# mjq11302010044/TPGSR

Hardware: AMD Instinct MI355X
Metric: training img/s (16x64->32x128, bs=48/GPU), TPGSR-TSRN full train step (higher is better)
Workload: dtype bf16x2; 1 GPU; C3: TPGSR-TSRN = TSRN_TL (STN+mask) + CRNN teacher/student text prior, stu_iter 1, full train step (teacher fwd, student fwd+bwd, distill loss, prior dropout, SR fwd+bwd, ImageLoss(gradient), clip 0.25, Adam); tpg=crnn, batch_per_gpu=48, global_batch=48, parallelism=dp1, launch=recorded plans, plain launches: main + weight-gradient + teacher streams

## Files before the change

### tpgsr_amd/csrc/conv_halo3.hip

```cpp
#include "conv_xbf_common.h"
#include <type_traits>

__device__ unsigned long long* g_halo3_trace = nullptr;
#define H3_STAMP(slot)                                                                                       \
  do {                                                                                                       \
    if (trace && lane == 0 && (slot) < 256)                                                                  \
      __builtin_nontemporal_store((unsigned long long)wall_clock64(), trace + (blockIdx.x * 8 + wave) * 256 + (slot)); \
  } while (0)

#define H3_TM 3
#define H3_NE 15
#define H3_PLANE (32 * H3_NE * 64)

template <int LD, int T, int TAPS>
__global__ __launch_bounds__(512, 2) void conv_halo3_xbf_kernel(tpgsr_conv_args a, int M, int Lcap) {
  extern __shared__ __attribute__((aligned(16))) unsigned char hsm[];
  constexpr int PLANE = H3_PLANE, BUF = T * PLANE;
  float* red_base = reinterpret_cast<float*>(hsm + 2 * BUF);
  float* stage_base = red_base + 2 * H3_TM * 256;
  const int tid = threadIdx.x;
  const int lane = tid & 63, wave = __builtin_amdgcn_readfirstlane(tid >> 6);
  typedef __attribute__((address_space(1))) unsigned long long* gptr_t;
  const gptr_t trace = blockIdx.x < 8 ? (gptr_t)g_halo3_trace : (gptr_t) nullptr;
  H3_STAMP(255);
  const int nbn = (a.Cout + 63) >> 6;
  const int mtiles = (M + 63) >> 6;
  const int nst = ((mtiles + H3_TM - 1) / H3_TM) * nbn;
  const int taps = a.KH * a.KW, NC = a.Cin >> 5;
  const int Hp = a.OH + a.KH - 1, Wp = a.OW + a.KW - 1, ohw = a.OH * a.OW;
  auto qbase = [&](int m) __attribute__((always_inline)) {
    const int n = m / ohw, r = m - n * ohw, oh = r / a.OW;
    return (n * Hp + oh) * Wp + (r - oh * a.OW);
  };

  if (wave >= 4) {
    const int pt = tid - 256, aq = pt & 7, er = pt >> 3;
    const __amdgpu_buffer_rsrc_t rs_in = make_rsrc(a.in, (size_t)a.N * a.H * a.W * a.in_ld);
    const __amdgpu_buffer_rsrc_t rs_in2 = make_rsrc(a.in2 ? a.in2 : a.in, (size_t)a.N * a.H * a.W * a.in2_ld);
    int hpix[H3_NE];
    auto decode_tile = [&](const int t) __attribute__((always_inline)) {
      const int m0 = (xcd_remap(t, nst) / nbn) * (64 * H3_TM);
      const int q0 = qbase(m0);
      const int L = qbase(min(m0 + 64 * H3_TM - 1, M - 1)) - q0 + (a.KH - 1) * Wp + a.KW;
      const int q = q0 + er * H3_NE;
      int n = q / (Hp * Wp);
      const int rem = q - n * (Hp * Wp);
      int r = rem / Wp, sx = rem - r * Wp;
#pragma unroll
      for (int i = 0; i < H3_NE; ++i) {
        const int ih = r - a.pad_h, iw = sx - a.pad_w;
        const bool in = n < a.N && (unsigned)ih < (unsigned)a.H && (unsigned)iw < (unsigned)a.W;
        hpix[i] = er * H3_NE + i < L ? (in ? (n * a.H + ih) * a.W + iw : -1) : -2;
        const bool c1 = ++sx >= Wp;
        sx = c1 ? 0 : sx;
        r += c1 ? 1 : 0;
        const bool c2 = r >= Hp;
        r = c2 ? 0 : r;
        n += c2 ? 1 : 0;
      }
    };
    constexpr bool DB = !(LD & 4);
    ARaw hr[DB ? 2 : 1][H3_NE];
    float4 qs[2], qt[2], q2 = make_float4(1.f, 1.f, 1.f, 1.f);
    qs[0] = qs[1] = make_float4(1.f, 1.f, 1.f, 1.f);
    qt[0] = qt[1] = make_float4(0.f, 0.f, 0.f, 0.f);
    auto load_item = [&](auto set_tag, const int cc) __attribute__((always_inline)) {
      constexpr int S = decltype(set_tag)::value;
      const int c = cc * 32 + aq * 4;
#pragma unroll
      for (int i = 0; i < H3_NE; ++i) {
        const bool ok = hpix[i] >= 0;
        hr[S][i].ok = (LD & 3) ? ok : true;
        hr[S][i].raw = false;
        hr[S][i].v = buf_load4(rs_in, ok ? ((unsigned)hpix[i] * (unsigned)a.in_ld + (unsigned)(a.in_coff + c)) * 4u : OOB_OFF);
        if (LD & 4) hr[S][i].v2 = buf_load4(rs_in2, ok ? ((unsigned)hpix[i] * (unsigned)a.in2_ld + (unsigned)c) * 4u : OOB_OFF);
      }
      if (LD & 1) {
        qs[S] = *reinterpret_cast<const float4*>(a.in_scale + c);
        qt[S] = *reinterpret_cast<const float4*>(a.in_shift + c);
      }
      if (LD & 32) q2 = *reinterpret_cast<const float4*>(a.in2_scale + c);
    };
    auto store_item = [&](auto set_tag, const int j) __attribute__((always_inline)) {
      constexpr int S = decltype(set_tag)::value;
      unsigned char* buf = hsm + (j & 1) * BUF;
#pragma unroll
      for (int i = 0; i < H3_NE; ++i) {
        const float4 v = finish_a<LD>(a, hr[S][i], qs[S], qt[S], q2);
        uint2 h[T];
        split4<T>(v, h);
        const int e = er * H3_NE + i;
        const int off = e * 64 + (((aq >> 1) ^ ((e >> 2) & 3)) << 4) + (aq & 1) * 8;
#pragma unroll
        for (int t = 0; t < T; ++t) *reinterpret_cast<uint2*>(buf + t * PLANE + off) = h[t];
      }
    };
    int t = blockIdx.x, cc = 0, j = 0;
    using P0 = std::integral_constant<int, 0>;
    using PN = std::integral_constant<int, DB ? 1 : 0>;
    decode_tile(t);
    if (DB) load_item(P0{}, 0);
    auto item = [&](auto cur_tag, auto nxt_tag) __attribute__((always_inline)) -> bool {
      int ncc = cc + 1, nt = t;
      if (ncc == NC) {
        ncc = 0;
        nt = t + gridDim.x;
      }
      const bool more = nt < nst;
      if (!DB) load_item(cur_tag, cc);
      if (more && ncc == 0) decode_tile(nt);
      if (DB && more) load_item(nxt_tag, ncc);
      H3_STAMP(4 * j);
      store_item(cur_tag, j);
      H3_STAMP(4 * j + 1);
      __syncthreads();
      H3_STAMP(4 * j + 2);
      ++j;
      t = nt;
      cc = ncc;
      return more;
    };
    while (true) {
      if (!item(P0{}, PN{})) break;
      if (!item(PN{}, P0{})) break;
    }
    __syncthreads();
    return;
  }

  {
  const int wm = wave & 1, wn = wave >> 1;
  const int wrows = a.wt_ld > 0 ? a.wt_ld : a.Cout;
  const int NB32 = (wrows + 31) >> 5, KB16 = a.kp >> 4;
  const __amdgpu_buffer_rsrc_t rs_w = make_rsrc(reinterpret_cast<const float*>(a.wt_bf), (size_t)T * NB32 * 32 * a.kp / 2);
  const unsigned plane_w = (unsigned)NB32 * KB16 * 1024u;
  const int g = lane >> 5;
  unsigned woff = 0;
  int ebase[H3_TM];

  floatx16 acc[H3_TM][1][1];
  bf16x8 av[2][H3_TM][T];
  u32x4 bw[2][2][T];
  int gtap = 0;
  auto fetch_w = [&](auto set_tag, auto kb_tag, const int tapidx) __attribute__((always_inline)) {
    constexpr int S = decltype(set_tag)::value, KB = decltype(kb_tag)::value;
#pragma unroll
    for (int t = 0; t < T; ++t)
      bw[S][KB][t] = __builtin_amdgcn_raw_buffer_load_b128(rs_w, (int)woff, (int)(t * plane_w + (unsigned)(2 * tapidx + KB) * 1024u), 0);
  };
  int an[H3_TM];
  auto addr_a = [&](auto kb_tag, const int bufoff, const int tapoff) __attribute__((always_inline)) {
    constexpr int KB = decltype(kb_tag)::value;
#pragma unroll
    for (int m = 0; m < H3_TM; ++m) {
      const int e = ebase[m] + tapoff;
      an[m] = bufoff + e * 64 + (((KB * 2 + g) ^ ((e >> 2) & 3)) << 4);
    }
  };
  auto read_a = [&](auto kb_tag) __attribute__((always_inline)) {
    constexpr int KB = decltype(kb_tag)::value;
#pragma unroll
    for (int m = 0; m < H3_TM; ++m)
#pragma unroll
      for (int t = 0; t < T; ++t) av[KB][m][t] = *reinterpret_cast<const bf16x8*>(hsm + an[m] + t * PLANE);
  };
  auto multiply = [&](auto set_tag, auto kb_tag) __attribute__((always_inline)) {
    constexpr int S = decltype(set_tag)::value, KB = decltype(kb_tag)::value;
    bf16x8 bv[T];
#pragma unroll
    for (int t = 0; t < T; ++t) bv[t] = __builtin_bit_cast(bf16x8, bw[S][KB][t]);
    if (T == 2) {
#pragma unroll
      for (int m = 0; m < H3_TM; ++m) acc[m][0][0] = __builtin_amdgcn_mfma_f32_32x32x16_bf16(av[KB][m][0], bv[T - 1], acc[m][0][0], 0, 0, 0);
#pragma unroll
      for (int m = 0; m < H3_TM; ++m) acc[m][0][0] = __builtin_amdgcn_mfma_f32_32x32x16_bf16(av[KB][m][T - 1], bv[0], acc[m][0][0], 0, 0, 0);
    }
#pragma unroll
    for (int m = 0; m < H3_TM; ++m) acc[m][0][0] = __builtin_amdgcn_mfma_f32_32x32x16_bf16(av[KB][m][0], bv[0], acc[m][0][0], 0, 0, 0);
  };
  using I0 = std::integral_constant<int, 0>;
  using I1 = std::integral_constant<int, 1>;
  int kw = 0, tapoff = 0;
  auto next_tap = [&]() __attribute__((always_inline)) {
    const bool cw = ++kw == a.KW;
    tapoff += cw ? Wp - a.KW + 1 : 1;
    kw = cw ? 0 : kw;
    asm volatile("" : "+s"(tapoff));
  };
#define H3_SGB(mask, n) __builtin_amdgcn_sched_group_barrier(mask, n, 0)
  auto interleave = [&](const bool ds) __attribute__((always_inline)) {
    constexpr int NM = 3 * (2 * T - 1);
    int used = 0;
    if (ds) {
#pragma unroll
      for (int i = 0; i < 3; ++i) {
        H3_SGB(0x008, 1);
        H3_SGB(0x100, T);
      }
      used = 3;
    }
    H3_SGB(0x008, 1);
    H3_SGB(0x020, T);
    ++used;
#pragma unroll
    for (int i = 0; i < NM; ++i) {
      if (i >= NM - used) break;
      H3_SGB(0x008, 1);
      H3_SGB(0x002, 3);
    }
  };
  auto tap = [&](auto set_tag, auto next_tag, const int bufoff) __attribute__((always_inline)) {
    constexpr int S = decltype(set_tag)::value;
    constexpr bool NEXT = decltype(next_tag)::value != 0;
    using SX = std::integral_constant<int, S ^ 1>;
    __builtin_amdgcn_sched_barrier(0);
    read_a(I1{});
    fetch_w(SX{}, I1{}, gtap + 1);
    if (NEXT) {
      next_tap();
      addr_a(I0{}, bufoff, tapoff);
    }
    multiply(set_tag, I0{});
    interleave(true);
    __builtin_amdgcn_sched_barrier(0);
    if (NEXT) read_a(I0{});
    fetch_w(set_tag, I0{}, gtap + 2);
    if (NEXT) addr_a(I1{}, bufoff, tapoff);
    multiply(set_tag, I1{});
    interleave(NEXT);
    __builtin_amdgcn_sched_barrier(0);
    ++gtap;
  };
  auto run_block = [&](auto s0_tag, const int bufoff) __attribute__((always_inline)) {
    constexpr int S0 = decltype(s0_tag)::value;
    using A0 = std::integral_constant<int, S0>;
    using A1 = std::integral_constant<int, S0 ^ 1>;
    kw = 0;
    tapoff = 0;
    addr_a(I0{}, bufoff, 0);
    read_a(I0{});
    addr_a(I1{}, bufoff, 0);
    if constexpr (TAPS > 0) {
      auto unrolled = [&](auto seq) __attribute__((always_inline)) {
        [&]<int... I>(std::integer_sequence<int, I...>) __attribute__((always_inline)) {
          (tap(std::integral_constant<int, S0 ^ (I & 1)>{}, std::integral_constant<int, (I + 1 < TAPS) ? 1 : 0>{}, bufoff), ...);
        }(seq);
      };
      unrolled(std::make_integer_sequence<int, TAPS>{});
    } else {
      for (int tp = 0; tp + 2 < taps; tp += 2) {
        tap(A0{}, I1{}, bufoff);
        tap(A1{}, I1{}, bufoff);
      }
      tap(A0{}, I0{}, bufoff);
    }
  };
  int j = 0, pend_mblk = -1, pend_n0 = 0, ndone = 0;
  auto flush_pending = [&]() __attribute__((always_inline)) {
    if (pend_mblk >= 0) {
      if (a.bn_row_tiles == H3_TM) {
        if (tid < 64 && pend_n0 + tid < a.Cout) {
          float v0 = 0.f, v1 = 0.f;
#pragma unroll
          for (int m = 0; m < H3_TM; ++m)
            if ((pend_mblk + m) * 64 < M) {
              const float* red = red_base + (((ndone - 1) & 1) * H3_TM + m) * 256;
              v0 += red[tid] + red[128 + tid];
              v1 += red[64 + tid] + red[192 + tid];
            }
          float* dst = a.bn_partial + (size_t)(pend_mblk / H3_TM) * 2 * a.Cout;
          dst[pend_n0 + tid] = v0;
          dst[a.Cout + pend_n0 + tid] = v1;
        }
      } else {
#pragma unroll
        for (int m = 0; m < H3_TM; ++m)
          if ((pend_mblk + m) * 64 < M)
            xbf_bn_flush<1, 1>(a, M, pend_n0, pend_mblk + m, tid, red_base + (((ndone - 1) & 1) * H3_TM + m) * 256);
      }
      pend_mblk = -1;
    }
  };
  for (int st = blockIdx.x; st < nst; st += gridDim.x) {
    const int tile = xcd_remap(st, nst);
    const int mblk3 = tile / nbn;
    const int m0 = mblk3 * (64 * H3_TM), n0 = (tile - mblk3 * nbn) * 64;
    const int q0 = qbase(m0);
    const int ncol0 = n0 + wn * 32;
    woff = ncol0 < a.Cout ? ((unsigned)((a.wt_coff + ncol0) >> 5) * KB16) * 1024u + lane * 16u : OOB_OFF;
#pragma unroll
    for (int m = 0; m < H3_TM; ++m) {
      ebase[m] = qbase(min(m0 + 64 * m + wm * 32 + (lane & 31), M - 1)) - q0;
#pragma unroll
      for (int r = 0; r < 16; ++r) acc[m][0][0][r] = 0.f;
    }
    gtap = 0;
    fetch_w(I0{}, I0{}, 0);
    fetch_w(I0{}, I1{}, 0);
    fetch_w(I1{}, I0{}, 1);
    for (int cc = 0; cc < NC; cc += 2) {
      H3_STAMP(4 * j);
      __syncthreads();
      H3_STAMP(4 * j + 1);
      flush_pending();
      run_block(I0{}, (j & 1) * BUF);
      H3_STAMP(4 * j + 2);
      ++j;
      if (cc + 1 < NC) {
        H3_STAMP(4 * j);
        __syncthreads();
        H3_STAMP(4 * j + 1);
        run_block(I1{}, (j & 1) * BUF);
        H3_STAMP(4 * j + 2);
        ++j;
      }
    }
    const bool bnb = a.bnb_y != nullptr;
    const bool fast = !a.out_ps && (a.Cout & 3) == 0 && (a.out_ld & 3) == 0 && (a.out_coff & 3) == 0 && ((uintptr_t)a.out & 15) == 0 &&
                      (!bnb || ((uintptr_t)a.bnb_y & 15) == 0);
    const bool full3 = m0 + 64 * (H3_TM - 1) < M;
    if (fast && !bnb && a.out_act == TPGSR_ACT_NONE && full3) {
      const int cloc = wn * 32 + (lane & 31), n = n0 + cloc;
      const bool nvalid = n < a.Cout;
      const float bias = (a.bias && nvalid) ? a.bias[n] : 0.f;
      const int quad = lane & 7, nq = n0 + wn * 32 + quad * 4;
      auto stage = [&](auto m_tag, float* stg) __attribute__((always_inline)) {
        constexpr int m = decltype(m_tag)::value;
        float sum = 0.f, sq = 0.f;
#pragma unroll
        for (int r = 0; r < 16; ++r) {
          const float raw = acc[m][0][0][r];
          if (nvalid) {
            sum += raw;
            sq = __builtin_fmaf(raw, raw, sq);
          }
          stg[((r & 3) + 8 * (r >> 2) + 4 * (lane >> 5)) * 32 + (lane & 31)] = raw + bias;
        }
        if (a.bn_partial) {
          float* red = red_base + ((ndone & 1) * H3_TM + m) * 256;
          sum += __shfl_xor(sum, 32);
          sq += __shfl_xor(sq, 32);
          if (lane < 32) {
            red[(wm * 2 + 0) * 64 + cloc] = sum;
            red[(wm * 2 + 1) * 64 + cloc] = sq;
          }
        }
      };
      auto drain = [&](auto m_tag, const float* stg) __attribute__((always_inline)) {
        constexpr int m = decltype(m_tag)::value;
#pragma unroll
        for (int k = 0; k < 4; ++k) {
          const int row = 8 * k + (lane >> 3);
          const float4 q4 = *reinterpret_cast<const float4*>(stg + row * 32 + quad * 4);
          if (nq < a.Cout) *reinterpret_cast<float4*>(a.out + (size_t)(m0 + 64 * m + wm * 32 + row) * a.out_ld + a.out_coff + nq) = q4;
        }
      };
      float* s0 = stage_base + wave * 2048;
      float* s1 = s0 + 1024;
      using M0 = std::integral_constant<int, 0>;
      using M1 = std::integral_constant<int, 1>;
      using M2 = std::integral_constant<int, 2>;
      stage(M0{}, s0);
      stage(M1{}, s1);
      drain(M0{}, s0);
      stage(M2{}, s0);
      drain(M1{}, s1);
      drain(M2{}, s0);
    } else {
    const int cloc = wn * 32 + (lane & 31), n = n0 + cloc;
    const bool nvalid = n < a.Cout;
    const float bias = (a.bias && nvalid) ? a.bias[n] : 0.f;
    const int quad = lane & 7, nq = n0 + wn * 32 + quad * 4;
    float b_mu = 0.f, b_rs = 0.f, b_sc = 1.f, b_sh = 0.f;
    if (bnb && nvalid) {
      if (a.bn_partial) {
        b_mu = a.bnb_mean[n];
        b_rs = a.bnb_rstd[n];
      }
      if (a.bnb_act && a.bnb_scale) {
        b_sc = a.bnb_scale[n];
        b_sh = a.bnb_shift[n];
      }
    }
    float4 yq[4];
    auto load_y = [&](const int m, float4 (&dst)[4]) __attribute__((always_inline)) {
#pragma unroll
      for (int k = 0; k < 4; ++k) {
        const int mm = m0 + 64 * m + wm * 32 + 8 * k + (lane >> 3);
        dst[k] = (mm < M && nq < a.Cout) ? *reinterpret_cast<const float4*>(a.bnb_y + (size_t)mm * a.Cout + nq) : make_float4(0.f, 0.f, 0.f, 0.f);
      }
    };
    if (bnb && fast) load_y(0, yq);
#pragma clang loop unroll(disable)
    for (int m = 0; m < H3_TM; ++m) {
      if (m0 + 64 * m >= M) break;
      floatx16 tile[1][1];
#pragma unroll
      for (int r = 0; r < 16; ++r) tile[0][0][r] = m == 0 ? acc[0][0][0][r] : m == 1 ? acc[1][0][0][r] : acc[2][0][0][r];
      float* red = red_base + ((ndone & 1) * H3_TM + m) * 256;
      if (!fast) {
        xbf_store_tile<1, 1>(a, tile, M, m0 + 64 * m, n0, wm, wn, lane, red);
        continue;
      }
      float* stg = stage_base + wave * 2048;
      float yv[16];
      float4 ynx[4];
      if (bnb) {
        if (m + 1 < H3_TM) load_y(m + 1, ynx);
#pragma unroll
        for (int k = 0; k < 4; ++k) *reinterpret_cast<float4*>(stg + (8 * k + (lane >> 3)) * 32 + quad * 4) = yq[k];
#pragma unroll
        for (int r = 0; r < 16; ++r) yv[r] = stg[((r & 3) + 8 * (r >> 2) + 4 * (lane >> 5)) * 32 + (lane & 31)];
      }
      float sum = 0.f, sq = 0.f;
      float v[16];
#pragma unroll
      for (int r = 0; r < 16; ++r) {
        const int row = (r & 3) + 8 * (r >> 2) + 4 * (lane >> 5);
        const int mm = m0 + 64 * m + wm * 32 + row;
        float raw = tile[0][0][r];
        if (mm < M && nvalid) {
          if (bnb) {
            const float dz = xbf_bnb_elem(raw, yv[r], b_sc, b_sh, b_mu, b_rs, a.bnb_act, sum, sq);
            if (a.bnb_store_dz) raw = dz;
          } else {
            sum += raw;
            sq = __builtin_fmaf(raw, raw, sq);
          }
        }
        v[r] = raw + bias;
      }
      if (a.out_act != TPGSR_ACT_NONE) {
#pragma unroll
        for (int r = 0; r < 16; ++r) v[r] = apply_act(v[r], a.out_act);
      }
#pragma unroll
      for (int r = 0; r < 16; ++r) stg[((r & 3) + 8 * (r >> 2) + 4 * (lane >> 5)) * 32 + (lane & 31)] = v[r];
      if (a.bn_partial) {
        sum += __shfl_xor(sum, 32);
        sq += __shfl_xor(sq, 32);
        if (lane < 32) {
          red[(wm * 2 + 0) * 64 + cloc] = sum;
          red[(wm * 2 + 1) * 64 + cloc] = sq;
        }
      }
#pragma unroll
      for (int k = 0; k < 4; ++k) {
        const int row = 8 * k + (lane >> 3);
        const int mm = m0 + 64 * m + wm * 32 + row;
        const float4 q4 = *reinterpret_cast<const float4*>(stg + row * 32 + quad * 4);
        if (mm < M && nq < a.Cout) *reinterpret_cast<float4*>(a.out + (size_t)mm * a.out_ld + a.out_coff + nq) = q4;
      }
      if (bnb) {
#pragma unroll
        for (int k = 0; k < 4; ++k) yq[k] = ynx[k];
      }
    }
    }
    H3_STAMP(4 * (j - 1) + 3);
    if (a.bn_partial) {
      pend_mblk = mblk3 * H3_TM;
      pend_n0 = n0;
    }
    ++ndone;
  }
  __syncthreads();
  flush_pending();
  }
}

static_assert(H3_TM == kH3Tiles && H3_NE == kH3Entries, "conv_route.h sizes this kernel's halo and LDS");

extern "C" int tpgsr_halo3_trace(unsigned long long* buf) {
  if (hipMemcpyToSymbol(HIP_SYMBOL(g_halo3_trace), &buf, sizeof(buf)) != hipSuccess) {
    tpgsr_set_error("tpgsr_halo3_trace: hipMemcpyToSymbol failed");
    return TPGSR_ERR_LAUNCH;
  }
  return 0;
}

#define H3_LD_CASES(X) X(0) X(1) X(2) X(3) X(4) X(5) X(7) X(37)

int conv_halo3_xbf_launch(const tpgsr_conv_args* a, long long M, const tpgsr_conv_route_t& r, hipStream_t st) {
  const int T = a->terms, ld = r.ld, Lcap = r.lcap;
  TPGSR_CHECK_ARG(a->bn_row_tiles == 0 || a->bn_row_tiles == 1 || a->bn_row_tiles == H3_TM,
                  "tpgsr_conv_fwd(halo3): bn_row_tiles %d (0, 1 or %d)", a->bn_row_tiles, H3_TM);
  const size_t lds = r.lds_bytes;
  const long long nst = (long long)cdiv(cdiv(M, 64), H3_TM) * cdiv(a->Cout, 64);
  const void* fn = nullptr;
  const bool t9 = a->KH * a->KW == 9;
#define H3_CASE(B)                                                                                                                 \
  case B:                                                                                                                          \
    fn = T == 1 ? (t9 ? (const void*)conv_halo3_xbf_kernel<B, 1, 9> : (const void*)conv_halo3_xbf_kernel<B, 1, 0>)                 \
                : (t9 ? (const void*)conv_halo3_xbf_kernel<B, 2, 9> : (const void*)conv_halo3_xbf_kernel<B, 2, 0>);                \
    break;
  switch (ld) {
    H3_LD_CASES(H3_CASE)
    default: return unsupported_ld("tpgsr_conv_fwd", ld);
  }
#undef H3_CASE
  int dev = 0, cus = 0;
  if (hipGetDevice(&dev) != hipSuccess || hipDeviceGetAttribute(&cus, hipDeviceAttributeMultiprocessorCount, dev) != hipSuccess || cus < 1) {
    tpgsr_set_error("tpgsr_conv_fwd(halo3): device query failed");
    return TPGSR_ERR_LAUNCH;
  }
  const int rc = lds_opt_in(fn, lds, "tpgsr_conv_fwd(halo3)");
  if (rc) return rc;
  dim3 grid((unsigned)(nst < cus ? nst : cus));
  int Mi = (int)M, Lc = Lcap;
  tpgsr_conv_args args = *a;
  void* params[] = {&args, &Mi, &Lc};
  if (hipLaunchKernel(fn, grid, dim3(512), params, lds, st) != hipSuccess) {
    tpgsr_set_error("tpgsr_conv_fwd(halo3): launch failed: %s", hipGetErrorString(hipGetLastError()));
    return TPGSR_ERR_LAUNCH;
  }
  TPGSR_LAUNCH_CHECK("tpgsr_conv_fwd(bf16 MFMA, whole-CU halo)");
}

extern "C" int tpgsr_conv_halo3_xbf_launch(const tpgsr_conv_args* a, long long M, int ld, hipStream_t st) {
  (void)ld;
  const tpgsr_conv_route_t r = conv_fwd_route(a, M);
  if (r.kernel != TPGSR_CONV_XBF_HALO3) return 0;
  const int rc = conv_halo3_xbf_launch(a, M, r, st);
  return rc < 0 ? rc : 1;
}
```

### tpgsr_amd/csrc/conv_xbf_common.h

```cpp
#pragma once
#include "conv_loader.h"
#include "conv_launch.h"

typedef __bf16 bf16x8 __attribute__((ext_vector_type(8)));
typedef __bf16 bf16x4 __attribute__((ext_vector_type(4)));
typedef short s16x4 __attribute__((ext_vector_type(4)));
typedef __attribute__((address_space(3))) s16x4* lds_s16x4_ptr;

#define XW_ROW 192
#define XW_PLANE (32 * XW_ROW)

template <int T>
__device__ __forceinline__ void split_bf(float x, __bf16 (&h)[T]) {
  h[0] = (__bf16)x;
  if (T > 1) {
    float r = x - (float)h[0];
    h[1] = (__bf16)r;
    if (T > 2) h[2] = (__bf16)(r - (float)h[1]);
  }
}
template <int T>
__device__ __forceinline__ void split4(const float4& v, uint2 (&out)[T]) {
  __bf16 a[T], b[T], c[T], d[T];
  split_bf<T>(v.x, a);
  split_bf<T>(v.y, b);
  split_bf<T>(v.z, c);
  split_bf<T>(v.w, d);
#pragma unroll
  for (int t = 0; t < T; ++t) {
    bf16x4 q;
    q[0] = a[t]; q[1] = b[t]; q[2] = c[t]; q[3] = d[t];
    out[t] = __builtin_bit_cast(uint2, q);
  }
}

template <int T>
__device__ __forceinline__ floatx16 mfma_terms(const bf16x8 (&a)[T], const bf16x8 (&b)[T], floatx16 acc) {
  if (T == 3) {
    acc = __builtin_amdgcn_mfma_f32_32x32x16_bf16(a[0], b[2], acc, 0, 0, 0);
    acc = __builtin_amdgcn_mfma_f32_32x32x16_bf16(a[2], b[0], acc, 0, 0, 0);
    acc = __builtin_amdgcn_mfma_f32_32x32x16_bf16(a[1], b[1], acc, 0, 0, 0);
    acc = __builtin_amdgcn_mfma_f32_32x32x16_bf16(a[0], b[1], acc, 0, 0, 0);
    acc = __builtin_amdgcn_mfma_f32_32x32x16_bf16(a[1], b[0], acc, 0, 0, 0);
  }
  if (T == 2) {
    acc = __builtin_amdgcn_mfma_f32_32x32x16_bf16(a[0], b[1], acc, 0, 0, 0);
    acc = __builtin_amdgcn_mfma_f32_32x32x16_bf16(a[1], b[0], acc, 0, 0, 0);
  }
  return __builtin_amdgcn_mfma_f32_32x32x16_bf16(a[0], b[0], acc, 0, 0, 0);
}

#ifndef XBF_NT_STORE
#define XBF_NT_STORE 0
#endif
__device__ __forceinline__ float xbf_bnb_elem(float raw, float y, float sc, float sh, float mu, float rs, int act, float& s, float& ss) {
  const float dz = act ? raw * act_grad(__builtin_fmaf(y, sc, sh), act) : raw;
  s += dz;
  ss = __builtin_fmaf(dz * (y - mu), rs, ss);
  return dz;
}

template <int WMB, int WNB>
__device__ __forceinline__ void xbf_store_tile(const tpgsr_conv_args& a, floatx16 (&acc)[WMB][WNB], int M, int m0, int n0, int wm,
                                               int wn, int lane, float* red) {
  constexpr int BNT = 64 * WNB;
  const int ohw = a.OH * a.OW;
#pragma unroll
  for (int j = 0; j < WNB; ++j) {
    const int cloc = wn * 32 * WNB + 32 * j + (lane & 31);
    const int n = n0 + cloc;
    const bool nvalid = n < a.Cout;
    const float bias = (a.bias && nvalid) ? a.bias[n] : 0.f;
    float s = 0.f, ss = 0.f;
    const bool bnb = a.bnb_y != nullptr;
    float b_mu = 0.f, b_rs = 0.f, b_sc = 1.f, b_sh = 0.f;
    if (bnb && nvalid) {
      if (a.bn_partial) {
        b_mu = a.bnb_mean[n];
        b_rs = a.bnb_rstd[n];
      }
      if (a.bnb_act && a.bnb_scale) {
        b_sc = a.bnb_scale[n];
        b_sh = a.bnb_shift[n];
      }
    }
#pragma unroll
    for (int i = 0; i < WMB; ++i) {
      float yv[16];
      if (bnb) {
#pragma unroll
        for (int r = 0; r < 16; ++r) {
          const int m = m0 + wm * 32 * WMB + 32 * i + (r & 3) + 8 * (r >> 2) + 4 * (lane >> 5);
          yv[r] = (m < M && nvalid) ? a.bnb_y[(size_t)m * a.Cout + n] : 0.f;
        }
      }
#pragma unroll
      for (int r = 0; r < 16; ++r) {
        int row = (r & 3) + 8 * (r >> 2) + 4 * (lane >> 5);
        int m = m0 + wm * 32 * WMB + 32 * i + row;
        if (m < M && nvalid) {
          float raw = acc[i][j][r];
          if (bnb) {
            const float dz = xbf_bnb_elem(raw, yv[r], b_sc, b_sh, b_mu, b_rs, a.bnb_act, s, ss);
            if (a.bnb_store_dz) raw = dz;
          } else {
            s += raw;
            ss = __builtin_fmaf(raw, raw, ss);
          }
          float v = apply_act(raw + bias, a.out_act);
          if (!a.out_ps) {
            if (XBF_NT_STORE) __builtin_nontemporal_store(v, &a.out[(size_t)m * a.out_ld + a.out_coff + n]);
            else a.out[(size_t)m * a.out_ld + a.out_coff + n] = v;
          } else {
            int nn = m / ohw;
            int rem = m - nn * ohw;
            int oh = rem / a.OW, ow = rem - oh * a.OW;
            int cs = n >> 2, pi = (n >> 1) & 1, pj = n & 1;
            a.out[((size_t)(nn * 2 * a.OH + 2 * oh + pi) * (2 * a.OW) + 2 * ow + pj) * (a.Cout >> 2) + cs] = v;
          }
        }
      }
    }
    if (a.bn_partial) {
      s += __shfl_xor(s, 32);
      ss += __shfl_xor(ss, 32);
      if (lane < 32) {
        red[(wm * 2 + 0) * BNT + cloc] = s;
        red[(wm * 2 + 1) * BNT + cloc] = ss;
      }
    }
  }
}
template <int WMB, int WNB>
__device__ __forceinline__ void xbf_store_tile_wide(const tpgsr_conv_args& a, floatx16 (&acc)[WMB][WNB], int M, int m0, int n0, int wm,
                                                    int wn, int lane, float* red, float* stage) {
  const bool fast = stage != nullptr && !a.out_ps && !a.bnb_y && (a.Cout & 3) == 0 && (a.out_ld & 3) == 0 && (a.out_coff & 3) == 0 &&
                    ((uintptr_t)a.out & 15) == 0;
  if (!fast) {
    xbf_store_tile<WMB, WNB>(a, acc, M, m0, n0, wm, wn, lane, red);
    return;
  }
  constexpr int BNT = 64 * WNB;
  const int quad = lane & 7;
#pragma unroll
  for (int j = 0; j < WNB; ++j) {
    const int cloc = wn * 32 * WNB + 32 * j + (lane & 31);
    const int n = n0 + cloc;
    const bool nvalid = n < a.Cout;
    const float bias = (a.bias && nvalid) ? a.bias[n] : 0.f;
    const int nq = n0 + wn * 32 * WNB + 32 * j + quad * 4;
    float s = 0.f, ss = 0.f;
#pragma unroll
    for (int i = 0; i < WMB; ++i) {
      const int mrow0 = m0 + wm * 32 * WMB + 32 * i;
      float v[16];
#pragma unroll
      for (int r = 0; r < 16; ++r) {
        const int m = mrow0 + (r & 3) + 8 * (r >> 2) + 4 * (lane >> 5);
        const float raw = acc[i][j][r];
        if (m < M && nvalid) {
          s += raw;
          ss = __builtin_fmaf(raw, raw, ss);
        }
        v[r] = raw + bias;
      }
      if (a.out_act != TPGSR_ACT_NONE) {
#pragma unroll
        for (int r = 0; r < 16; ++r) v[r] = apply_act(v[r], a.out_act);
      }
#pragma unroll
      for (int r = 0; r < 16; ++r) stage[((r & 3) + 8 * (r >> 2) + 4 * (lane >> 5)) * 32 + (lane & 31)] = v[r];
#pragma unroll
      for (int k = 0; k < 4; ++k) {
        const int row = 8 * k + (lane >> 3);
        const int m = mrow0 + row;
        const float4 q4 = *reinterpret_cast<const float4*>(stage + row * 32 + quad * 4);
        if (m < M && nq < a.Cout) *reinterpret_cast<float4*>(a.out + (size_t)m * a.out_ld + a.out_coff + nq) = q4;
      }
    }
    if (a.bn_partial) {
      s += __shfl_xor(s, 32);
      ss += __shfl_xor(ss, 32);
      if (lane < 32) {
        red[(wm * 2 + 0) * BNT + cloc] = s;
        red[(wm * 2 + 1) * BNT + cloc] = ss;
      }
    }
  }
}

template <int WMB, int WNB>
__device__ __forceinline__ void xbf_bn_flush(const tpgsr_conv_args& a, int M, int n0, int mblk, int tid, const float* red) {
  constexpr int BNT = 64 * WNB;
  for (int e = tid; e < BNT * WMB; e += 256) {
    const int blk = e / BNT, c = e - blk * BNT;
    const long long rb64 = (long long)mblk * WMB + blk;
    if (n0 + c < a.Cout && rb64 * 64 < M) {
      float* dst = a.bn_partial + (size_t)rb64 * 2 * a.Cout;
      float v0, v1;
      if (WMB == 1) {
        v0 = red[0 * BNT + c] + red[2 * BNT + c];
        v1 = red[1 * BNT + c] + red[3 * BNT + c];
      } else {
        v0 = red[(blk * 2 + 0) * BNT + c];
        v1 = red[(blk * 2 + 1) * BNT + c];
      }
      dst[n0 + c] = v0;
      dst[a.Cout + n0 + c] = v1;
    }
  }
}

template <int WMB, int WNB>
__device__ __forceinline__ void xbf_epilogue(const tpgsr_conv_args& a, floatx16 (&acc)[WMB][WNB], int M, int m0, int n0, int mblk,
                                             int wm, int wn, int lane, int tid, float* red, float* stage = nullptr) {
  xbf_store_tile_wide<WMB, WNB>(a, acc, M, m0, n0, wm, wn, lane, red, stage);
  if (a.bn_partial) {
    __syncthreads();
    xbf_bn_flush<WMB, WNB>(a, M, n0, mblk, tid, red);
  }
}
```

Before: 9008 img/s.

## Precompute Mish-gradient factors in producer waves for halo3 BN-backward epilogue

Adds a PF variant of the halo3 conv kernel for T=2, 3x3 convs with a fused Mish-BN backward epilogue. On the last tile, the otherwise idle producer waves load the saved activations, compute the Mish derivative factor, and write it into a free halo LDS buffer. The MMA waves then read these factors instead of evaluating act_grad themselves, so the transcendental epilogue work overlaps with the main loop. In exchange, the producer waves do extra global loads and there is an extra barrier, and the fast path only applies to the final tile of each block and only under strict alignment conditions.

```diff
diff --git a/tpgsr_amd/csrc/conv_halo3.hip b/tpgsr_amd/csrc/conv_halo3.hip
--- a/tpgsr_amd/csrc/conv_halo3.hip
+++ b/tpgsr_amd/csrc/conv_halo3.hip
@@ -12,8 +12,9 @@
 #define H3_NE 15
 #define H3_PLANE (32 * H3_NE * 64)
 
-template <int LD, int T, int TAPS>
+template <int LD, int T, int TAPS, bool PF = false>
 __global__ __launch_bounds__(512, 2) void conv_halo3_xbf_kernel(tpgsr_conv_args a, int M, int Lcap) {
+  static_assert(!PF || (T == 2 && TAPS == 9 && H3_TM * 64 * 64 * 4 <= 2 * H3_PLANE), "the factor plane lives in one halo buffer");
   extern __shared__ __attribute__((aligned(16))) unsigned char hsm[];
   constexpr int PLANE = H3_PLANE, BUF = T * PLANE;
   float* red_base = reinterpret_cast<float*>(hsm + 2 * BUF);
@@ -32,6 +33,16 @@
     const int n = m / ohw, r = m - n * ohw, oh = r / a.OW;
     return (n * Hp + oh) * Wp + (r - oh * a.OW);
   };
+  auto pf_takes = [&](const int st, const int m0) __attribute__((always_inline)) -> bool {
+    return st + (int)gridDim.x >= nst && m0 + 64 * H3_TM <= M && a.bnb_y != nullptr && a.bnb_act == TPGSR_ACT_MISH &&
+           a.out_act == TPGSR_ACT_NONE && !a.out_ps && (a.Cout & 3) == 0 && (a.out_ld & 3) == 0 && (a.out_coff & 3) == 0 &&
+           ((uintptr_t)a.out & 15) == 0 && ((uintptr_t)a.bnb_y & 15) == 0 && (long long)M * a.Cout * 4 <= 0x7fffffffll;
+  };
+  auto pf_y = [&](const __amdgpu_buffer_rsrc_t rs_y, const unsigned voff, const int m, const int r) __attribute__((always_inline)) -> float {
+    return __uint_as_float(__builtin_amdgcn_raw_buffer_load_b32(rs_y, (int)voff, (64 * m + (r & 3) + 8 * (r >> 2)) * a.Cout * 4, 0));
+  };
+  (void)pf_y;
+  (void)pf_takes;
 
   if (wave >= 4) {
     const int pt = tid - 256, aq = pt & 7, er = pt >> 3;
@@ -95,6 +106,41 @@
         for (int t = 0; t < T; ++t) *reinterpret_cast<uint2*>(buf + t * PLANE + off) = h[t];
       }
     };
+    float fy[H3_TM][16];
+    float f_sc = 1.f, f_sh = 0.f;
+    auto pf_load_y = [&](const int st) __attribute__((always_inline)) -> bool {
+      const int tile = xcd_remap(st, nst);
+      const int mblk3 = tile / nbn;
+      const int m0 = mblk3 * (64 * H3_TM), n0 = (tile - mblk3 * nbn) * 64;
+      if (!pf_takes(st, m0)) return false;
+      const int pw = wave - 4;
+      const int n = n0 + (pw >> 1) * 32 + (lane & 31);
+      const bool nvalid = n < a.Cout;
+      const __amdgpu_buffer_rsrc_t rs_y = make_rsrc(a.bnb_y, (size_t)M * a.Cout);
+      const unsigned voff = nvalid ? ((unsigned)(m0 + (pw & 1) * 32 + 4 * (lane >> 5)) * (unsigned)a.Cout + (unsigned)n) * 4u : OOB_OFF;
+#pragma unroll
+      for (int m = 0; m < H3_TM; ++m)
+#pragma unroll
+        for (int r = 0; r < 16; ++r) fy[m][r] = pf_y(rs_y, voff, m, r);
+      if (nvalid && a.bnb_scale) {
+        f_sc = a.bnb_scale[n];
+        f_sh = a.bnb_shift[n];
+      }
+      return true;
+    };
+    auto pf_store_f = [&](const int jl) __attribute__((always_inline)) {
+      float4* fpl = reinterpret_cast<float4*>(hsm + ((jl & 1) ^ 1) * BUF) + (wave - 4) * 64 + lane;
+#pragma unroll
+      for (int m = 0; m < H3_TM; ++m) {
+        float f[16];
+#pragma unroll
+        for (int r = 0; r < 16; ++r) f[r] = act_grad(__builtin_fmaf(fy[m][r], f_sc, f_sh), TPGSR_ACT_MISH);
+#pragma unroll
+        for (int k = 0; k < 4; ++k) fpl[(m * 4 + k) * 256] = make_float4(f[4 * k], f[4 * k + 1], f[4 * k + 2], f[4 * k + 3]);
+      }
+    };
+    (void)pf_load_y;
+    (void)pf_store_f;
     int t = blockIdx.x, cc = 0, j = 0;
     using P0 = std::integral_constant<int, 0>;
     using PN = std::integral_constant<int, DB ? 1 : 0>;
@@ -113,6 +159,9 @@
       H3_STAMP(4 * j);
       store_item(cur_tag, j);
       H3_STAMP(4 * j + 1);
+      if constexpr (PF) {
+        if (!more) return false;
+      }
       __syncthreads();
       H3_STAMP(4 * j + 2);
       ++j;
@@ -123,6 +172,16 @@
     while (true) {
       if (!item(P0{}, PN{})) break;
       if (!item(PN{}, P0{})) break;
+    }
+    if constexpr (PF) {
+      const bool pf = pf_load_y(t);
+      __syncthreads();
+      H3_STAMP(4 * j + 2);
+      if (pf) {
+        pf_store_f(j);
+        __syncthreads();
+        H3_STAMP(4 * j + 3);
+      }
     }
     __syncthreads();
     return;
@@ -319,7 +378,72 @@
     const bool fast = !a.out_ps && (a.Cout & 3) == 0 && (a.out_ld & 3) == 0 && (a.out_coff & 3) == 0 && ((uintptr_t)a.out & 15) == 0 &&
                       (!bnb || ((uintptr_t)a.bnb_y & 15) == 0);
     const bool full3 = m0 + 64 * (H3_TM - 1) < M;
-    if (fast && !bnb && a.out_act == TPGSR_ACT_NONE && full3) {
+    bool pf = false;
+    if constexpr (PF) pf = pf_takes(st, m0);
+    if (pf) {
+      const int cloc = wn * 32 + (lane & 31), n = n0 + cloc;
+      const bool nvalid = n < a.Cout;
+      const float bias = (a.bias && nvalid) ? a.bias[n] : 0.f;
+      const int quad = lane & 7, nq = n0 + wn * 32 + quad * 4;
+      float b_mu = 0.f, b_rs = 0.f;
+      if (nvalid && a.bn_partial) {
+        b_mu = a.bnb_mean[n];
+        b_rs = a.bnb_rstd[n];
+      }
+      float yv[H3_TM][16];
+      const __amdgpu_buffer_rsrc_t rs_y = make_rsrc(a.bnb_y, (size_t)M * a.Cout);
+      const unsigned voff = nvalid ? ((unsigned)(m0 + wm * 32 + 4 * (lane >> 5)) * (unsigned)a.Cout + (unsigned)n) * 4u : OOB_OFF;
+#pragma unroll
+      for (int m = 0; m < H3_TM; ++m)
+#pragma unroll
+        for (int r = 0; r < 16; ++r) yv[m][r] = pf_y(rs_y, voff, m, r);
+      __syncthreads();
+      const float4* fpl = reinterpret_cast<const float4*>(hsm + (j & 1) * BUF) + wave * 64 + lane;
+      auto stage = [&](auto m_tag, float* stg) __attribute__((always_inline)) {
+        constexpr int m = decltype(m_tag)::value;
+        float4 fq[4];
+#pragma unroll
+        for (int k = 0; k < 4; ++k) fq[k] = fpl[(m * 4 + k) * 256];
+        float sum = 0.f, sq = 0.f;
+#pragma unroll
+        for (int r = 0; r < 16; ++r) {
+          float raw = acc[m][0][0][r];
+          const float f = (r & 3) == 0 ? fq[r >> 2].x : (r & 3) == 1 ? fq[r >> 2].y : (r & 3) == 2 ? fq[r >> 2].z : fq[r >> 2].w;
+          const float dz = xbf_bnb_elem_f(raw, yv[m][r], f, b_mu, b_rs, sum, sq);
+          if (a.bnb_store_dz) raw = dz;
+          stg[((r & 3) + 8 * (r >> 2) + 4 * (lane >> 5)) * 32 + (lane & 31)] = raw + bias;
+        }
+        if (a.bn_partial) {
+          float* red = red_base + ((ndone & 1) * H3_TM + m) * 256;
+          sum += __shfl_xor(sum, 32);
+          sq += __shfl_xor(sq, 32);
+          if (lane < 32) {
+            red[(wm * 2 + 0) * 64 + cloc] = sum;
+            red[(wm * 2 + 1) * 64 + cloc] = sq;
+          }
+        }
+      };
+      auto drain = [&](auto m_tag, const float* stg) __attribute__((always_inline)) {
+        constexpr int m = decltype(m_tag)::value;
+#pragma unroll
+        for (int k = 0; k < 4; ++k) {
+          const int row = 8 * k + (lane >> 3);
+          const float4 q4 = *reinterpret_cast<const float4*>(stg + row * 32 + quad * 4);
+          if (nq < a.Cout) *reinterpret_cast<float4*>(a.out + (size_t)(m0 + 64 * m + wm * 32 + row) * a.out_ld + a.out_coff + nq) = q4;
+        }
+      };
+      float* s0 = stage_base + wave * 2048;
+      float* s1 = s0 + 1024;
+      using M0 = std::integral_constant<int, 0>;
+      using M1 = std::integral_constant<int, 1>;
+      using M2 = std::integral_constant<int, 2>;
+      stage(M0{}, s0);
+      stage(M1{}, s1);
+      drain(M0{}, s0);
+      stage(M2{}, s0);
+      drain(M1{}, s1);
+      drain(M2{}, s0);
+    } else if (fast && !bnb && a.out_act == TPGSR_ACT_NONE && full3) {
       const int cloc = wn * 32 + (lane & 31), n = n0 + cloc;
       const bool nvalid = n < a.Cout;
       const float bias = (a.bias && nvalid) ? a.bias[n] : 0.f;
@@ -489,9 +613,11 @@
   const long long nst = (long long)cdiv(cdiv(M, 64), H3_TM) * cdiv(a->Cout, 64);
   const void* fn = nullptr;
   const bool t9 = a->KH * a->KW == 9;
+  const bool pf = T == 2 && t9 && a->bnb_y && a->bnb_act != TPGSR_ACT_NONE && a->out_act == TPGSR_ACT_NONE && !a->out_ps;
 #define H3_CASE(B)                                                                                                                 \
   case B:                                                                                                                          \
-    fn = T == 1 ? (t9 ? (const void*)conv_halo3_xbf_kernel<B, 1, 9> : (const void*)conv_halo3_xbf_kernel<B, 1, 0>)                 \
+    fn = pf     ? (const void*)conv_halo3_xbf_kernel<B, 2, 9, true>                                                                \
+       : T == 1 ? (t9 ? (const void*)conv_halo3_xbf_kernel<B, 1, 9> : (const void*)conv_halo3_xbf_kernel<B, 1, 0>)                 \
                 : (t9 ? (const void*)conv_halo3_xbf_kernel<B, 2, 9> : (const void*)conv_halo3_xbf_kernel<B, 2, 0>);                \
     break;
   switch (ld) {
diff --git a/tpgsr_amd/csrc/conv_xbf_common.h b/tpgsr_amd/csrc/conv_xbf_common.h
--- a/tpgsr_amd/csrc/conv_xbf_common.h
+++ b/tpgsr_amd/csrc/conv_xbf_common.h
@@ -55,6 +55,13 @@
 #endif
 __device__ __forceinline__ float xbf_bnb_elem(float raw, float y, float sc, float sh, float mu, float rs, int act, float& s, float& ss) {
   const float dz = act ? raw * act_grad(__builtin_fmaf(y, sc, sh), act) : raw;
+  s += dz;
+  ss = __builtin_fmaf(dz * (y - mu), rs, ss);
+  return dz;
+}
+__device__ __forceinline__ float xbf_bnb_elem_f(float raw, float y, float f, float mu, float rs, float& s, float& ss) {
+#pragma clang fp contract(off)
+  const float dz = raw * f;
   s += dz;
   ss = __builtin_fmaf(dz * (y - mu), rs, ss);
   return dz;
```

Result: no change. 9039 img/s (median of 6 runs) (+0.3%).
